# rapidsai/cugraph-gnn

Hardware: AMD Instinct MI355X
Metric: sampled-edges/sec (sample+renumber+feature-gather+SAGEConv fwd), ogbn-products-like fan-out [25, 10] (higher is better)
Workload: dtype int64 ids (int32 timed as a variant) + f32 features (SAGE lin_l/lin_r product: bf16x3-split MFMA, f32 accumulate); 1 GPU; ogbn-products-like RMAT: V=2449029, E=118462496 directed (CSR row_ptr i64 / col i64 replicated per GPU), feat fp32 [V,100], batch 1024/GPU, fan-out [25, 10], 2-layer SAGEConv(mean) 100-256-47 fwd, step = 8 call groups of 188 mini-batches; parallelism=dp1 (seeds sharded, no data-path collective)

## Files before the change

cugraph-gnn_amd/csrc/wg_sage_mfma.hip:

```cpp
#include "wg_sage_mfma_parts.hpp"

namespace wgamd {
namespace {
using namespace sage_mfma;

template <int TR>
__device__ __forceinline__ void consume_tile(const mfma_args& a, int64_t tile, const float* tile_lds, int cw, int lane,
                                             float* scratch)
{
  constexpr int RT = TR / 32;
  f32x16 c[RT][2];
#pragma unroll
  for (int rt = 0; rt < RT; rt++)
#pragma unroll
    for (int ct = 0; ct < 2; ct++)
#pragma unroll
      for (int i = 0; i < 16; i++) c[rt][ct][i] = 0.f;
  const int lm = lane & 31, lh = lane >> 5;
  const float* a_lane      = tile_lds + lm * a.SD + lh * 8;
  const float* b_lane = a.w_tiles + ((int64_t)(cw * 64 + lm)) * 16 + lh * 8;
  braw_t b0, b1;
  bfrag_t fb;
  araw_t<RT> raw;
  afrag_t<RT> fa;
  load_b(b0, b_lane, a.N, 0);
  for (int ks = 0; ks < a.KS; ks += 2) {
    load_a_raw<RT>(raw, a_lane, a.SD, ks);
    if (ks + 1 < a.KS) load_b(b1, b_lane, a.N, ks + 1);
    split_a<RT>(raw, fa);
    split_b(b0, fb);
    mma_frags<RT>(c, fa, fb);
    if (ks + 1 < a.KS) {
      load_a_raw<RT>(raw, a_lane, a.SD, ks + 1);
      if (ks + 2 < a.KS) load_b(b0, b_lane, a.N, ks + 2);
      split_a<RT>(raw, fa);
      split_b(b1, fb);
      mma_frags<RT>(c, fa, fb);
    }
  }
  epilogue<RT>(a, c, tile * TR, cw, lane, scratch);
}

template <int HEAD, int BODY, int VALU_PER>
__device__ __forceinline__ void mfma_valu_interleave()
{
#pragma unroll
  for (int i = 0; i < HEAD; i++) __builtin_amdgcn_sched_group_barrier(0x008, 1, 0);
#pragma unroll
  for (int i = 0; i < BODY; i++) {
    __builtin_amdgcn_sched_group_barrier(0x008, 1, 0);
    __builtin_amdgcn_sched_group_barrier(0x002, VALU_PER, 0);
  }
}

template <int RT, int AD, typename RawT = araw_t<RT>, typename LoadA>
__device__ __forceinline__ void consume_range(const mfma_args& a, f32x16 (&c)[RT][2], bfrag_t (&b)[3], int ks0, int ks1, int cw,
                                              int lane, LoadA load_a)
{
  const int lm = lane & 31, lh = lane >> 5;
  const int64_t b_plane_dw = (int64_t)a.KS * a.N * 8;
  const uint32_t* b_lane   = reinterpret_cast<const uint32_t*>(a.w_tiles) + ((int64_t)(cw * 64 + lm)) * 8 + lh * 4;
  RawT raw[AD];
  afrag_t<RT> fa[2];
  const int kl = ks1 - 1;
  load_a(raw[0], ks0);
  if constexpr (AD == 2) load_a(raw[1], ks0 + 1 < kl ? ks0 + 1 : kl);
  split_raw<RT>(raw[0], fa[0]);
  auto step = [&](auto I, int ks) {
    constexpr int i = decltype(I)::value;
    load_a(raw[i % AD], ks + AD < kl ? ks + AD : kl);
    int kb = ks + 2;
    kb     = kb >= a.KS ? kb - a.KS : kb;
    load_b_planes(b[(i + 2) % 3], b_lane, b_plane_dw, a.N, kb);
    mma_frags<RT>(c, fa[i & 1], b[i % 3]);
    split_raw<RT>(raw[(i + 1) % AD], fa[(i + 1) & 1]);
    mfma_valu_interleave<4, 6 * RT * 2 - 4, 5>();
    __builtin_amdgcn_sched_barrier(0);
  };
  int ks = ks0;
  for (; ks + 5 < ks1; ks += 6) {
    step(std::integral_constant<int, 0>{}, ks);
    step(std::integral_constant<int, 1>{}, ks + 1);
    step(std::integral_constant<int, 2>{}, ks + 2);
    step(std::integral_constant<int, 3>{}, ks + 3);
    step(std::integral_constant<int, 4>{}, ks + 4);
    step(std::integral_constant<int, 5>{}, ks + 5);
  }
  const int r = ks1 - ks;
  if (r > 0) step(std::integral_constant<int, 0>{}, ks);
  if (r > 1) step(std::integral_constant<int, 1>{}, ks + 1);
  if (r > 2) step(std::integral_constant<int, 2>{}, ks + 2);
  if (r > 3) step(std::integral_constant<int, 3>{}, ks + 3);
  if (r > 4) step(std::integral_constant<int, 4>{}, ks + 4);
  const int rot = (ks1 - ks0) % 3;
  if (rot == 1) {
    const bfrag_t t = b[0];
    b[0] = b[1], b[1] = b[2], b[2] = t;
  } else if (rot == 2) {
    const bfrag_t t = b[0];
    b[0] = b[2], b[2] = b[1], b[1] = t;
  }
}

constexpr int kPD = 2;
__host__ __device__ constexpr int b_slot(int ks) { return ks < kPD ? ks : kPD + (ks % kPD); }
__host__ __device__ constexpr int w_lds_ksteps(int FC)
{
#ifdef WG_NO_WLDS
  return 0;
#endif
  const int tiles = (2 * 64 * row_stride_dw(FC) + 16 + 4 * kScratchDw + 16) * 4;
  const int free_ = 160 * 1024 - tiles;
  const int ks    = free_ / (256 * 64);
  return ks < 0 ? 0 : (ks > 4 ? 4 : ks);
}

template <int TR, int FC>
struct static_consumer {
  static constexpr int RT = TR / 32, KSC = (2 * FC + 15) / 16, SD = row_stride_dw(FC);
  static constexpr int KL = TR == 64 ? w_lds_ksteps(FC) : 0;
  braw_t bb[2 * kPD];
  uint32_t b_lane_off;
  const float* w_lds;
  f32x16 c[RT][2];

  __device__ __forceinline__ void load_b_static(const mfma_args& a, braw_t& f, int ks) const
  {
#ifdef WG_ABL_NO_B
    return;
#endif
#ifdef WG_ABL_HALF_B
    if (ks & 1) return;
#endif
    if (ks >= KSC - KL) {
#pragma unroll
      for (int ct = 0; ct < 2; ct++)
#pragma unroll
        for (int h = 0; h < 2; h++)
          f.v[ct][h] = *reinterpret_cast<const f32x4*>(w_lds + (((ks - (KSC - KL)) * 2 + ct) * 2 + h) * 256);
      return;
    }
    const char* wb = reinterpret_cast<const char*>(a.w_tiles);
#pragma unroll
    for (int ct = 0; ct < 2; ct++) {
      const size_t at = ((size_t)ks * a.N + ct * 32) * 64 + b_lane_off;
      f.v[ct][0]      = *reinterpret_cast<const f32x4*>(wb + at);
      f.v[ct][1]      = *reinterpret_cast<const f32x4*>(wb + at + 16);
    }
  }

  __device__ __forceinline__ void prime(const mfma_args& a, int cw, int lane, float* w_lds_wave)
  {
    b_lane_off = (uint32_t)(((cw * 64 + (lane & 31)) * 16 + (lane >> 5) * 8) * 4);
    w_lds      = w_lds_wave + lane * 4;
    if constexpr (KL > 0) {
      const char* wb = reinterpret_cast<const char*>(a.w_tiles);
#pragma unroll
      for (int ks = KSC - KL; ks < KSC; ks++)
#pragma unroll
        for (int ct = 0; ct < 2; ct++)
#pragma unroll
          for (int h = 0; h < 2; h++)
            *reinterpret_cast<f32x4*>(const_cast<float*>(w_lds) + (((ks - (KSC - KL)) * 2 + ct) * 2 + h) * 256) =
              *reinterpret_cast<const f32x4*>(wb + ((size_t)ks * a.N + ct * 32) * 64 + b_lane_off + h * 16);
    }
#pragma unroll
    for (int j = 0; j < kPD; j++) load_b_static(a, bb[j], j);
  }

  __device__ __forceinline__ void multiply(const mfma_args& a, const float* tile_lds, int lane)
  {
#pragma unroll
    for (int rt = 0; rt < RT; rt++)
#pragma unroll
      for (int ct = 0; ct < 2; ct++)
#pragma unroll
        for (int i = 0; i < 16; i++) c[rt][ct][i] = 0.f;
    const float* a_lane = tile_lds + (lane & 31) * SD + (lane >> 5) * 8;
    araw_t<RT> raw;
    afrag_t<RT> fa[2];
    load_a_raw<RT>(raw, a_lane, SD, 0);
    split_a<RT>(raw, fa[0]);
#pragma unroll
    for (int ks = 0; ks < KSC; ks++) {
      if (ks + 1 < KSC) load_a_raw<RT>(raw, a_lane, SD, ks + 1);
      bfrag_t fb;
      split_b(bb[b_slot(ks)], fb);
      mma_frags<RT>(c, fa[ks & 1], fb);
      const int nk = ks + kPD;
      if (nk < KSC) load_b_static(a, bb[b_slot(nk)], nk);
      else load_b_static(a, bb[nk - KSC], nk - KSC);
      if (ks + 1 < KSC) split_a<RT>(raw, fa[(ks + 1) & 1]);
      __builtin_amdgcn_sched_barrier(0);
    }
  }
  __device__ __forceinline__ void store(const mfma_args& a, int64_t tile, int cw, int lane, float* scratch)
  {
    epilogue<RT>(a, c, tile * TR, cw, lane, scratch);
  }
};

template <typename IdT, int LG, int TR, int CW, bool OFF32, int FC, bool HALF = false, typename XT = float>
__global__ void __launch_bounds__((CW + kProducerWaves) * 64)
sage_layer_mfma_kernel(mfma_args a)
{
  static_assert(!HALF || FC == 0, "the half-tile mode runs the runtime-shape consumer");
  extern __shared__ __attribute__((aligned(16))) float lds[];
  const int tile_dw = TR * a.SD;
  uint32_t* ring = reinterpret_cast<uint32_t*>(lds + 2 * tile_dw + 16 + CW * kScratchDw) + 8;
  uint32_t first_ticket = kNoTile;
  if (threadIdx.x == 0 && (int64_t)blockIdx.x < (a.n_rows + TR - 1) / TR) first_ticket = (uint32_t)gridDim.x + atomicAdd(a.tickets, 1u);
  for (int i = threadIdx.x; i < 2 * tile_dw + 16; i += blockDim.x) lds[i] = 0.f;
  if (threadIdx.x == 0) ring[0] = blockIdx.x, ring[1] = first_ticket;
  __syncthreads();
  const int lane = threadIdx.x & 63;
  int wave = threadIdx.x >> 6;
  if (a.debug & 64) {
    uint32_t* keys = reinterpret_cast<uint32_t*>(lds + 2 * tile_dw + 16 + CW * kScratchDw);
    const int simd = (int)__builtin_amdgcn_s_getreg((1 << 11) | (4 << 6) | 4);
    if (lane == 0) keys[wave] = (uint32_t)(((simd & 1) * 2 + (simd >> 1)) * 16 + wave);
    __syncthreads();
    const uint32_t mine_key = keys[wave];
    int rank = 0;
#pragma unroll
    for (int w = 0; w < CW + kProducerWaves; w++) rank += keys[w] < mine_key ? 1 : 0;
    wave = __builtin_amdgcn_readfirstlane(rank);
    __syncthreads();
  }
  const uint32_t n_tiles = (uint32_t)((a.n_rows + TR - 1) / TR);
  const bool drawer      = wave == CW && lane == 0;
  auto draw              = [&](uint32_t known) {
    return known < n_tiles ? (uint32_t)gridDim.x + atomicAdd(a.tickets, 1u) : kNoTile;
  };
  auto ring_at = [&](int r) { return (uint32_t)__builtin_amdgcn_readfirstlane((int)ring[r]); };
  uint32_t t_prev = kNoTile, t_cur = ring_at(0);
  int r_next = 1;
  auto advance = [&](uint32_t t_next) {
    t_prev = t_cur, t_cur = t_next;
    r_next = r_next == 2 ? 0 : r_next + 1;
  };
  auto r_draw = [&] { return r_next == 2 ? 0 : r_next + 1; };
  auto stamp            = [&](int64_t n, int which) {
    if (a.stamps && blockIdx.x == 0 && lane == 0 && n < 64) a.stamps[(n * 8 + wave) * 2 + which] = __builtin_readcyclecounter();
  };

  if constexpr (HALF) {
    const int KSh = a.KS / 2;
    if (wave >= CW) {
      using P     = producer<IdT, LG, 32, OFF32, true, XT>;
      using off_t = typename P::off_t;
      constexpr int IT = P::IT, kNb = P::kNb, kDepth = P::kDepth;
      static_assert(TR == 64, "two 32-row sub-tiles per tile");
      P p(a, wave - CW, lane);
      bounds_t<IT> b_next;
      ids_t<IT> i_next;
      meta_t<IT, off_t> cur;
      typename P::raw_t buf[kDepth][kNb + 1];
      p.load_bounds(2 * (int64_t)t_cur, b_next);
      p.load_ids(2 * (int64_t)t_cur, b_next, i_next);
      p.finish(i_next, cur);
#pragma unroll
      for (int it = 0; it < kDepth - 1; it++) p.issue(cur, it, buf[it]);
      constexpr int kHalf = IT / 2;
      for (int n = 0;; n++) {
        const uint32_t t_next = ring_at(r_next);
        uint32_t drawn       = kNoTile;
        if (drawer && t_cur < n_tiles) drawn = draw(t_next);
        if (t_cur < n_tiles && !(a.debug & 2)) {
          float* tile_lds = lds + (n & 1) * tile_dw;
#pragma unroll
          for (int sub = 0; sub < 2; sub++) {
            const int64_t s_cur = 2 * (int64_t)t_cur + sub, s_next = sub == 0 ? s_cur + 1 : 2 * (int64_t)t_next;
            float* rows_lds = tile_lds + sub * 32 * a.SD;
            p.load_bounds(s_next, b_next);
#pragma unroll
            for (int it = 0; it < IT; it++) {
              if (it == kHalf) p.load_ids(s_next, b_next, i_next);
              if (it + kDepth - 1 < IT) p.issue(cur, it + kDepth - 1, buf[(it + kDepth - 1) % kDepth]);
              p.reduce_store(cur, it, buf[it % kDepth], rows_lds);
            }
            p.second_window(cur, rows_lds);
            p.long_rows(s_cur, cur, rows_lds);
            if (sub == 1 && drawer) ring[r_draw()] = drawn;
            p.finish(i_next, cur);
            if (sub == 0 || t_next < n_tiles) {
#pragma unroll
              for (int it = 0; it < kDepth - 1; it++) p.issue(cur, it, buf[it]);
            }
          }
        } else if (drawer) ring[r_draw()] = drawn;
        lds_barrier();
        if (t_cur >= n_tiles) break;
        advance(t_next);
      }
    } else {
      constexpr int RT = TR / 32;
      float* scratch = lds + 2 * tile_dw + 16 + wave * kScratchDw;
      f32x16 c[RT][2];
      bfrag_t b[3];
      {
        const uint32_t* b_lane =
          reinterpret_cast<const uint32_t*>(a.w_tiles) + ((int64_t)(wave * 64 + (lane & 31))) * 8 + (lane >> 5) * 4;
        load_b_planes(b[0], b_lane, (int64_t)a.KS * a.N * 8, a.N, 0);
        load_b_planes(b[1], b_lane, (int64_t)a.KS * a.N * 8, a.N, 1);
      }
      const IdT* src_ids = static_cast<const IdT*>(a.src_ids);
      for (int n = 0;; n++) {
        const uint32_t t_next = ring_at(r_next);
        if (n >= 1 && !(a.debug & 1)) {
          const int64_t row0 = (int64_t)t_prev * TR;
          constexpr int kEB = x16::row_elems<XT>::kBytes;
          using self_t      = typename std::conditional<kEB == 4, float, uint16_t>::type;
          const self_t* self_ptr[RT];
#pragma unroll
          for (int rt = 0; rt < RT; rt++) {
            const int64_t row  = row0 + rt * 32 + (lane & 31);
            const int64_t srow = a.self_rows[row < a.n_rows ? row : a.n_rows - 1];
            self_ptr[rt]       = reinterpret_cast<const self_t*>(reinterpret_cast<const char*>(a.x) + table_row<IdT>(src_ids, srow) * a.row_scale) +
                           (lane >> 5) * 8;
          }
#pragma unroll
          for (int rt = 0; rt < RT; rt++)
#pragma unroll
            for (int ct = 0; ct < 2; ct++)
#pragma unroll
              for (int i = 0; i < 16; i++) c[rt][ct][i] = 0.f;
          store_agg<TR, CW>(a, lds + ((n - 1) & 1) * tile_dw, row0, wave, lane);
          const float* a_lane = lds + ((n - 1) & 1) * tile_dw + (lane & 31) * a.SD + (lane >> 5) * 8;
          consume_range<RT, 1>(a, c, b, 0, KSh, wave, lane, [&](araw_t<RT>& f, int ks) { load_a_raw<RT>(f, a_lane, a.SD, ks); });
          if constexpr (kEB == 4) {
            consume_range<RT, 2>(a, c, b, KSh, a.KS, wave, lane, [&](araw_t<RT>& f, int ks) {
#pragma unroll
              for (int rt = 0; rt < RT; rt++) {
                const float* p = self_ptr[rt] + (ks - KSh) * 16;
                f.v[rt][0]     = *reinterpret_cast<const f32x4*>(p);
                f.v[rt][1]     = *reinterpret_cast<const f32x4*>(p + 4);
              }
            });
          } else {
            consume_range<RT, 2, araw16_t<XT, RT>>(a, c, b, KSh, a.KS, wave, lane, [&](araw16_t<XT, RT>& f, int ks) {
#pragma unroll
              for (int rt = 0; rt < RT; rt++)
                f.v[rt] = *reinterpret_cast<const x16::u32x4_a8*>(self_ptr[rt] + (ks - KSh) * 16);
            });
          }
          epilogue<RT>(a, c, row0, wave, lane, scratch);
        }
        lds_barrier();
        if (t_cur >= n_tiles) break;
        advance(t_next);
      }
    }
  } else if (wave >= CW) {
    if (a.debug & 16) __builtin_amdgcn_s_setprio(3);
    using P     = producer<IdT, LG, TR, OFF32, false, XT>;
    using off_t = typename P::off_t;
    constexpr int IT = P::IT, kNb = P::kNb, kDepth = P::kDepth;
    P p(a, wave - CW, lane);
    bounds_t<IT> b_next;
    ids_t<IT> i_next;
    meta_t<IT, off_t> cur;
    typename P::raw_t buf[kDepth][kNb + 1];
    {
      p.load_bounds(t_cur, b_next);
      p.load_ids(t_cur, b_next, i_next);
      p.finish(i_next, cur);
    }
#pragma unroll
    for (int it = 0; it < kDepth - 1; it++) p.issue(cur, it, buf[it]);
    constexpr int kHalf = IT / 2;
    for (int n = 0;; n++) {
      stamp(n, 0);
      const uint32_t t_next = ring_at(r_next);
      uint32_t drawn       = kNoTile;
      if (drawer && t_cur < n_tiles) drawn = draw(t_next);
      if (t_cur < n_tiles && !(a.debug & 2)) {
        float* tile_lds = lds + (n & 1) * tile_dw;
        p.load_bounds(t_next, b_next);
#pragma unroll
        for (int it = 0; it < IT; it++) {
          if (it == kHalf) p.load_ids(t_next, b_next, i_next);
          if (it + kDepth - 1 < IT) p.issue(cur, it + kDepth - 1, buf[(it + kDepth - 1) % kDepth]);
          p.reduce_store(cur, it, buf[it % kDepth], tile_lds);
        }
        p.second_window(cur, tile_lds);
        p.long_rows(t_cur, cur, tile_lds);
        if (drawer) ring[r_draw()] = drawn;
        p.finish(i_next, cur);
        if (t_next < n_tiles) {
#pragma unroll
          for (int it = 0; it < kDepth - 1; it++) p.issue(cur, it, buf[it]);
        }
      } else if (drawer) ring[r_draw()] = drawn;
      stamp(n, 1);
      lds_barrier();
      if (t_cur >= n_tiles) break;
      advance(t_next);
    }
  } else {
    if (a.debug & 32) __builtin_amdgcn_s_setprio(3);
    float* scratch = lds + 2 * tile_dw + 16 + wave * kScratchDw;
    if constexpr (FC > 0) {
      static_consumer<TR, FC> cons;
      cons.prime(a, wave, lane, lds + 2 * tile_dw + 16 + CW * kScratchDw + 16 + wave * (decltype(cons)::KL * 16 * 64));
      const bool late = (wave & 1) && !(a.debug & 128);
      int64_t pending = -1;
      for (int n = 0;; n++) {
        stamp(n, 0);
        const uint32_t t_next = ring_at(r_next);
        if (n >= 1 && !(a.debug & 1)) {
          const float* tile_lds = lds + ((n - 1) & 1) * tile_dw;
          store_agg<TR, CW>(a, tile_lds, (int64_t)t_prev * TR, wave, lane);
          if (late) {
            if (pending >= 0) cons.store(a, pending, wave, lane, scratch);
            cons.multiply(a, tile_lds, lane);
            pending = t_prev;
          } else {
            cons.multiply(a, tile_lds, lane);
            cons.store(a, t_prev, wave, lane, scratch);
          }
        }
        stamp(n, 1);
        lds_barrier();
        if (t_cur >= n_tiles) break;
        advance(t_next);
      }
      if (late && pending >= 0) cons.store(a, pending, wave, lane, scratch);
    } else {
      for (int n = 0;; n++) {
        const uint32_t t_next = ring_at(r_next);
        if (n >= 1 && !(a.debug & 1)) {
          store_agg<TR, CW>(a, lds + ((n - 1) & 1) * tile_dw, (int64_t)t_prev * TR, wave, lane);
          consume_tile<TR>(a, t_prev, lds + ((n - 1) & 1) * tile_dw, wave, lane, scratch);
        }
        lds_barrier();
        if (t_cur >= n_tiles) break;
        advance(t_next);
      }
    }
  }
  if (threadIdx.x == 0 && atomicAdd(a.tickets + 1, 1u) == gridDim.x - 1) {
    atomicExch(a.tickets, 0u);
    atomicExch(a.tickets + 1, 0u);
  }
}

__global__ void split_weight_kernel(const float* __restrict__ w_t, int64_t ldw, int K, int N, int KS, uint32_t* __restrict__ planes)
{
  const int64_t total = (int64_t)KS * N * 8;
  for (int64_t i = blockIdx.x * (int64_t)blockDim.x + threadIdx.x; i < total; i += (int64_t)gridDim.x * blockDim.x) {
    const int kk2 = (int)(i & 7);
    const int n   = (int)((i >> 3) % N);
    const int ks  = (int)((i >> 3) / N);
    const int k0  = ks * 16 + kk2 * 2;
    const float v0 = k0 < K ? w_t[(int64_t)k0 * ldw + n] : 0.f;
    const float v1 = k0 + 1 < K ? w_t[(int64_t)(k0 + 1) * ldw + n] : 0.f;
    uint32_t h0, m0, l0, h1, m1, l1;
    split3(v0, h0, m0, l0);
    split3(v1, h1, m1, l1);
    planes[i]             = pack_hi16(h0, h1);
    planes[total + i]     = pack_hi16(m0, m1);
    planes[2 * total + i] = pack_hi16(l0, l1);
  }
}

__global__ void tile_weight_kernel(const float* __restrict__ w_t, int64_t ldw, int K, int N, int KS, float* __restrict__ tiles)
{
  const int64_t total = (int64_t)KS * N * 16;
  for (int64_t i = blockIdx.x * (int64_t)blockDim.x + threadIdx.x; i < total; i += (int64_t)gridDim.x * blockDim.x) {
    const int kk = (int)(i & 15);
    const int n  = (int)((i >> 4) % N);
    const int ks = (int)((i >> 4) / N);
    const int k  = ks * 16 + kk;
    tiles[i]     = k < K ? w_t[(int64_t)k * ldw + n] : 0.f;
  }
}

__global__ void layer_weight_kernel(const float* __restrict__ w_l, int64_t ldl, const float* __restrict__ w_r, int64_t ldr,
                                    const float* __restrict__ bias, int F, int N, int Np, int KS, int half,
                                    void* __restrict__ planes_, float* __restrict__ bias_out)
{
  auto w_at = [&](int k, int n) -> float {
    if (n >= N || k >= 2 * F) return 0.f;
    return k < F ? w_l[(int64_t)n * ldl + k] : w_r[(int64_t)n * ldr + (k - F)];
  };
  const int64_t tid = blockIdx.x * (int64_t)blockDim.x + threadIdx.x, stride = (int64_t)gridDim.x * blockDim.x;
  if (bias_out)
    for (int64_t n = tid; n < Np; n += stride) bias_out[n] = (bias && n < N) ? bias[n] : 0.f;
  if (half) {
    uint32_t* planes    = static_cast<uint32_t*>(planes_);
    const int64_t total = (int64_t)KS * Np * 8;
    for (int64_t i = tid; i < total; i += stride) {
      const int kk2 = (int)(i & 7), n = (int)((i >> 3) % Np), ks = (int)((i >> 3) / Np);
      const int k0  = ks * 16 + kk2 * 2;
      uint32_t h0, m0, l0, h1, m1, l1;
      split3(w_at(k0, n), h0, m0, l0);
      split3(w_at(k0 + 1, n), h1, m1, l1);
      planes[i]             = pack_hi16(h0, h1);
      planes[total + i]     = pack_hi16(m0, m1);
      planes[2 * total + i] = pack_hi16(l0, l1);
    }
  } else {
    float* tiles        = static_cast<float*>(planes_);
    const int64_t total = (int64_t)KS * Np * 16;
    for (int64_t i = tid; i < total; i += stride) {
      const int kk = (int)(i & 15), n = (int)((i >> 4) % Np), ks = (int)((i >> 4) / Np);
      tiles[i]     = w_at(ks * 16 + kk, n);
    }
  }
}

constexpr int kSlotsPerBlock = 512;
__host__ inline uint32_t* ticket_slot(hipStream_t st)
{
  struct key_t {
    int dev;
    hipStream_t st;
    unsigned long long capture;
    bool operator<(const key_t& o) const { return std::tie(dev, st, capture) < std::tie(o.dev, o.st, o.capture); }
  };
  struct block_t {
    uint32_t* base;
    int used;
  };
  static std::mutex m;
  static std::map<key_t, uint32_t*> slot_of;
  static std::map<int, block_t> block_of;
  key_t key{0, st, 0};
  WG_HIP_CHECK(hipGetDevice(&key.dev));
  hipStreamCaptureStatus status = hipStreamCaptureStatusNone;
  if (st != nullptr) WG_HIP_CHECK(hipStreamGetCaptureInfo(st, &status, &key.capture));
  if (status != hipStreamCaptureStatusActive) key.capture = 0;
  std::lock_guard<std::mutex> g(m);
  auto it = slot_of.find(key);
  if (it != slot_of.end()) return it->second;
  block_t& b = block_of[key.dev];
  if (b.base == nullptr || b.used == kSlotsPerBlock) {
    hipStreamCaptureMode mode = hipStreamCaptureModeRelaxed;
    WG_HIP_CHECK(hipThreadExchangeStreamCaptureMode(&mode));
    void* p             = nullptr;
    const hipError_t e1 = hipMalloc(&p, kSlotsPerBlock * 2 * sizeof(uint32_t));
    const hipError_t e2 = e1 == hipSuccess ? hipMemset(p, 0, kSlotsPerBlock * 2 * sizeof(uint32_t)) : e1;
    WG_HIP_CHECK(hipThreadExchangeStreamCaptureMode(&mode));
    WG_HIP_CHECK(e1);
    WG_HIP_CHECK(e2);
    b = block_t{static_cast<uint32_t*>(p), 0};
  }
  uint32_t* slot = b.base + 2 * b.used++;
  slot_of.emplace(key, slot);
  return slot;
}

constexpr size_t kLdsBudget = 160 * 1024;
__host__ inline size_t lds_bytes(int F, int TR) { return (size_t)(2 * TR * row_stride_dw(F) + 16 + 4 * kScratchDw + 16) * 4; }
__host__ inline size_t lds_bytes_half(int F) { return (size_t)(2 * 64 * row_stride_half_dw(F) + 16 + 4 * kScratchDw + 16) * 4; }
__host__ inline bool use_half_tiles(int F)
{
  return F % 16 == 0 && lds_bytes(F, 64) > kLdsBudget && lds_bytes_half(F) <= kLdsBudget;
}

template <typename IdT, int LG, int CW, typename XT = float>
void launch_half(mfma_args a, hipStream_t st)
{
  const int cus         = stream_cu_count(st);
  a.tickets             = ticket_slot(st);
  a.SD                  = row_stride_half_dw(a.F);
  const int64_t n_tiles = (a.n_rows + 63) / 64;
  const size_t lds      = lds_bytes_half(a.F);
  const int grid        = (int)std::max<int64_t>(1, std::min<int64_t>(n_tiles, (int64_t)cus));
  auto go               = [&](auto kern) {
    WG_HIP_CHECK(hipFuncSetAttribute(reinterpret_cast<const void*>(kern), hipFuncAttributeMaxDynamicSharedMemorySize, (int)lds));
    kern<<<grid, (CW + kProducerWaves) * 64, lds, st>>>(a);
    WG_HIP_CHECK(hipGetLastError());
  };
  if (a.x_bytes != 0) go(sage_layer_mfma_kernel<IdT, LG, 64, CW, true, 0, true, XT>);
  else go(sage_layer_mfma_kernel<IdT, LG, 64, CW, false, 0, true, XT>);
}

template <typename IdT, int LG, int TR, int CW, int FC = 0, typename XT = float>
void launch(mfma_args a, hipStream_t st)
{
  const int cus         = stream_cu_count(st);
  a.tickets             = ticket_slot(st);
  const int64_t n_tiles = (a.n_rows + TR - 1) / TR;
  const size_t lds      = lds_bytes(a.F, TR) + (FC > 0 && TR == 64 ? (size_t)w_lds_ksteps(FC) * CW * 64 * 64 : 0);
  const int grid = (int)std::max<int64_t>(1, std::min<int64_t>(n_tiles, (int64_t)cus));
  auto go        = [&](auto kern) {
    if (lds > 64 * 1024)
      WG_HIP_CHECK(hipFuncSetAttribute(reinterpret_cast<const void*>(kern), hipFuncAttributeMaxDynamicSharedMemorySize, (int)lds));
    kern<<<grid, (CW + kProducerWaves) * 64, lds, st>>>(a);
    WG_HIP_CHECK(hipGetLastError());
  };
  if (a.x_bytes != 0) go(sage_layer_mfma_kernel<IdT, LG, TR, CW, true, FC, false, XT>);
  else go(sage_layer_mfma_kernel<IdT, LG, TR, CW, false, FC, false, XT>);
}

template <typename IdT, int LG, int TR, typename XT = float>
void launch_cw(const mfma_args& a, hipStream_t st)
{
  switch (a.N / 64) {
    case 1: launch<IdT, LG, TR, 1, 0, XT>(a, st); break;
    case 2: launch<IdT, LG, TR, 2, 0, XT>(a, st); break;
    default:
      if constexpr (LG == 32 && TR == 64) {
        if (a.F == 100) return launch<IdT, LG, TR, 4, 100, XT>(a, st);
        if (a.F == 128) return launch<IdT, LG, TR, 4, 128, XT>(a, st);
      }
      launch<IdT, LG, TR, 4, 0, XT>(a, st);
      break;
  }
}

template <typename IdT, int LG, typename XT = float>
void launch_tr(const mfma_args& a, hipStream_t st)
{
  if constexpr (LG <= 32) {
    launch_cw<IdT, LG, 64, XT>(a, st);
  } else {
    if (use_half_tiles(a.F) && !a.full_tiles) {
      switch (a.N / 64) {
        case 1: launch_half<IdT, LG, 1, XT>(a, st); break;
        case 2: launch_half<IdT, LG, 2, XT>(a, st); break;
        default: launch_half<IdT, LG, 4, XT>(a, st); break;
      }
    } else launch_cw<IdT, LG, 32, XT>(a, st);
  }
}

template <typename IdT, typename XT = float>
void launch_groups(const mfma_args& a, hipStream_t st)
{
  const int units = a.F / 4;
  if (units <= 8) launch_tr<IdT, 8, XT>(a, st);
  else if (units <= 16) launch_tr<IdT, 16, XT>(a, st);
  else if (units <= 32) launch_tr<IdT, 32, XT>(a, st);
  else launch_tr<IdT, 64, XT>(a, st);
}

}

namespace sage_mfma {
void launch_f16(const mfma_args& a, int ids_bytes, hipStream_t st);
void launch_bf16(const mfma_args& a, int ids_bytes, hipStream_t st);
#ifdef WG_SAGE_X16_TYPE
void WG_SAGE_X16_LAUNCH(const mfma_args& a, int ids_bytes, hipStream_t st)
{
  if (ids_bytes == 0) launch_groups<void, WG_SAGE_X16_TYPE>(a, st);
  else if (ids_bytes == 4) launch_groups<int32_t, WG_SAGE_X16_TYPE>(a, st);
  else launch_groups<int64_t, WG_SAGE_X16_TYPE>(a, st);
}
#endif
}
}

#if !defined(WG_MFMA_TUNE_HARNESS) && !defined(WG_SAGE_X16_TYPE)
extern "C" size_t wgamd_sage_weight_planes_bytes(int K, int N) { return (size_t)3 * ((K + 15) / 16) * (size_t)N * 32; }

extern "C" int wgamd_sage_layer_bf16x3_supported(int F, int N)
{
  return F > 0 && F % 4 == 0 && F <= 256 && (N == 64 || N == 128 || N == 256) && wgamd::lds_bytes(F, 32) <= wgamd::kLdsBudget;
}

extern "C" wholememory_error_code_t wgamd_sage_split_weight_bf16x3(const float* w_t, int64_t ldw, int K, int N, void* planes,
                                                                   void* stream)
{
  using namespace wgamd;
  return guarded("wgamd_sage_split_weight_bf16x3", [&] {
    WG_REQUIRE_INPUT(w_t && planes && K > 0 && N > 0 && ldw >= N, "bad weight");
    const int KS        = (K + 15) / 16;
    const int64_t total = (int64_t)KS * N * 16;
    const int grid      = (int)std::min<int64_t>((total + 255) / 256, 2048);
    if (K % 2 == 0 && use_half_tiles(K / 2))
      split_weight_kernel<<<grid, 256, 0, static_cast<hipStream_t>(stream)>>>(w_t, ldw, K, N, KS, static_cast<uint32_t*>(planes));
    else
      tile_weight_kernel<<<grid, 256, 0, static_cast<hipStream_t>(stream)>>>(w_t, ldw, K, N, KS, static_cast<float*>(planes));
    WG_HIP_CHECK(hipGetLastError());
  });
}

extern "C" int wgamd_sage_layer_uses_half_tiles(int F) { return wgamd::use_half_tiles(F) ? 1 : 0; }

extern "C" wholememory_error_code_t wgamd_sage_layer_weight_planes(const float* w_l, int64_t ldl, const float* w_r, int64_t ldr,
                                                                  const float* bias, int F, int N, int Np, void* planes,
                                                                  float* bias_out, int full_tiles, void* stream)
{
  using namespace wgamd;
  return guarded("wgamd_sage_layer_weight_planes", [&] {
    WG_REQUIRE_INPUT(w_l && w_r && planes && F > 0 && N > 0 && Np >= N && ldl >= F && ldr >= F, "bad weights");
    const int K = 2 * F, KS = (K + 15) / 16;
    const int half      = (use_half_tiles(F) && !full_tiles) ? 1 : 0;
    const int64_t total = (int64_t)KS * Np * 16;
    const int grid      = (int)std::min<int64_t>((total + 255) / 256, 2048);
    layer_weight_kernel<<<grid, 256, 0, static_cast<hipStream_t>(stream)>>>(w_l, ldl, w_r, ldr, bias, F, N, Np, KS, half, planes, bias_out);
    WG_HIP_CHECK(hipGetLastError());
  });
}

extern "C" wholememory_error_code_t wgamd_sage_layer_fused_bf16x3(const int* row_ptr, const int* col, int64_t n_rows,
                                                                  const float* x, int64_t ldx, int64_t x_rows, int F,
                                                                  const void* src_ids, wholememory_dtype_t src_ids_dtype,
                                                                  const int64_t* self_rows, int mean, const void* w_planes,
                                                                  int N, const float* bias, int relu, float* out, int64_t ldo,
                                                                  void* stream)
{
  return wgamd_sage_layer_fused_bf16x3_x_train(row_ptr, col, n_rows, x, WHOLEMEMORY_DT_FLOAT, ldx, x_rows, F, src_ids, src_ids_dtype,
                                               self_rows, mean, w_planes, N, bias, relu, out, ldo, nullptr, 0, stream);
}

extern "C" wholememory_error_code_t wgamd_sage_layer_fused_bf16x3_train(const int* row_ptr, const int* col, int64_t n_rows,
                                                                        const float* x, int64_t ldx, int64_t x_rows, int F,
                                                                        const void* src_ids, wholememory_dtype_t src_ids_dtype,
                                                                        const int64_t* self_rows, int mean, const void* w_planes,
                                                                        int N, const float* bias, int relu, float* out,
                                                                        int64_t ldo, float* agg_out, int64_t ld_agg, void* stream)
{
  return wgamd_sage_layer_fused_bf16x3_x_train(row_ptr, col, n_rows, x, WHOLEMEMORY_DT_FLOAT, ldx, x_rows, F, src_ids, src_ids_dtype,
                                               self_rows, mean, w_planes, N, bias, relu, out, ldo, agg_out, ld_agg, stream);
}

extern "C" int wgamd_sage_layer_x16_supported(int F, int N, wholememory_dtype_t x_dtype)
{
  return (x_dtype == WHOLEMEMORY_DT_FLOAT || x_dtype == WHOLEMEMORY_DT_HALF || x_dtype == WHOLEMEMORY_DT_BF16) &&
         wgamd_sage_layer_bf16x3_supported(F, N);
}

extern "C" wholememory_error_code_t wgamd_sage_layer_fused_bf16x3_x(const int* row_ptr, const int* col, int64_t n_rows,
                                                                    const void* x, wholememory_dtype_t x_dtype, int64_t ldx,
                                                                    int64_t x_rows, int F, const void* src_ids,
                                                                    wholememory_dtype_t src_ids_dtype, const int64_t* self_rows,
// ... 60 lines not shown
```

cugraph-gnn_amd/csrc/wg_sage_mfma_parts.hpp:

```cpp
#pragma once
#include <algorithm>
#include <cstdlib>
#include <map>
#include <mutex>
#include <tuple>
#include <type_traits>

#include "wg_common.hpp"
#include "wgamd_ext.h"
#include "wg_x16.hpp"

namespace wgamd {
namespace sage_mfma {

using f32x4  = __attribute__((ext_vector_type(4))) float;
using f32x16 = __attribute__((ext_vector_type(16))) float;
using u32x4  = __attribute__((ext_vector_type(4))) uint32_t;
using bf16x8 = __attribute__((ext_vector_type(8))) __bf16;

#ifndef WG_MFMA_PRODUCTS
#define WG_MFMA_PRODUCTS 6
#endif
#ifndef WG_MFMA_DEPTH
#define WG_MFMA_DEPTH 2
// ... 234 lines not shown
  {
    if constexpr (k < kNb + (HALF ? 0 : 1)) {
      issue_one<k>(m, it, v);
      issue_all<k + 1>(m, it, v);
    }
  }
  template <int k>
  __device__ __forceinline__ void issue_one(const meta_t<IT, off_t>& m, int it, raw_t* v) const
  {
    static_assert(!HALF || k < kNb, "no self slot in half-tile mode");
    if constexpr (OFF32) {
      if constexpr (k < kNb) {
        const uint32_t off = (uint32_t)group_lane<k>((int)m.src[it]);
        v[k] = bload(k < m.d[it] ? off + f0c * kEB : a.x_bytes);
      } else {
        v[kNb] = bload(m.d[it] >= 0 ? (uint32_t)m.self[it] + f0c * kEB : a.x_bytes);
      }
    } else {
      const char* xb = reinterpret_cast<const char*>(a.x);
      if constexpr (k < kNb) {
        const int lo = group_lane<k>((int)(m.src[it] & 0xffffffff));
        const int hi = group_lane<k>((int)((int64_t)m.src[it] >> 32));
        int64_t off  = ((int64_t)hi << 32) | (uint32_t)lo;
        off          = k < m.d[it] ? off : (int64_t)0;
        v[k]         = gload(xb + off + f0c * kEB);
      } else {
        v[kNb] = gload(xb + (m.d[it] >= 0 ? (int64_t)m.self[it] : (int64_t)0) + f0c * kEB);
      }
    }
  }
  __device__ __forceinline__ void reduce_store(const meta_t<IT, off_t>& m, int it, const raw_t* v, float* tile_lds) const
  {
    const int deg = m.d[it];
    f32x4 acc     = {0.f, 0.f, 0.f, 0.f};
#pragma unroll
    for (int k = 0; k < kNb; k++) {
      if constexpr (OFF32) acc += E::f32(v[k]);
      else acc += k < deg ? E::f32(v[k]) : f32x4{0.f, 0.f, 0.f, 0.f};
    }
    if (a.mean && deg > 0 && deg <= kNb) acc *= __frcp_rn((float)deg);
    if (live) {
      float* prow = tile_lds + (group + it * kGroups) * a.SD;
      *reinterpret_cast<f32x4*>(prow + f0) = acc;
      if constexpr (!HALF) {
        f32x4 self = E::f32(v[kNb]);
        if constexpr (!OFF32) self = deg >= 0 ? self : f32x4{0.f, 0.f, 0.f, 0.f};
        *reinterpret_cast<f32x4*>(prow + a.F + f0) = self;
      }
    }
  }
  static constexpr int kW2 = LG >= 32 ? 16 : (LG > kNb ? LG - kNb : 0);
  __device__ __forceinline__ void second_window(const meta_t<IT, off_t>& m, float* tile_lds) const
  {
    if constexpr (kW2 > 0) {
#pragma unroll
      for (int it = 0; it < IT; it++) {
        const int deg = m.d[it];
        if (__ballot(deg > kNb) == 0ull) continue;
        const bool mine = live && deg > kNb;
        raw_t v[kW2];
#pragma unroll
        for (int k = 0; k < kW2; k++) {
          const int kk = kNb + k;
          if constexpr (OFF32) {
            const uint32_t off = (uint32_t)__shfl((int)m.src[it], gbase | kk, 64);
            v[k] = bload(kk < deg ? off + f0c * kEB : a.x_bytes);
          } else {
            const int lo = __shfl((int)(m.src[it] & 0xffffffff), gbase | kk, 64);
            const int hi = __shfl((int)((int64_t)m.src[it] >> 32), gbase | kk, 64);
            int64_t off  = ((int64_t)hi << 32) | (uint32_t)lo;
            off          = kk < deg ? off : (int64_t)0;
            v[k]         = gload(reinterpret_cast<const char*>(a.x) + off + f0c * kEB);
          }
        }
        float* prow = tile_lds + (group + it * kGroups) * a.SD + f0;
        f32x4 acc   = {0.f, 0.f, 0.f, 0.f};
        if (mine) acc = *reinterpret_cast<const f32x4*>(prow);
#pragma unroll
        for (int k = 0; k < kW2; k++) {
          if constexpr (OFF32) acc += E::f32(v[k]);
          else acc += kNb + k < deg ? E::f32(v[k]) : f32x4{0.f, 0.f, 0.f, 0.f};
        }
        if (mine) {
          if (a.mean && deg <= kNb + kW2) acc *= __frcp_rn((float)deg);
          *reinterpret_cast<f32x4*>(prow) = acc;
        }
      }
    }
  }
  static constexpr int kLongUnroll = 8;
  __device__ __forceinline__ void long_rows(int64_t tile, const meta_t<IT, off_t>& m, float* tile_lds) const
  {
    long_rows_from<kNb + kW2, kLongUnroll>(tile, m, tile_lds);
  }
  template <int kStart, int kUnroll>
  __device__ __forceinline__ void long_rows_from(int64_t tile, const meta_t<IT, off_t>& m, float* tile_lds) const
  {
    const IdT* src_ids = static_cast<const IdT*>(a.src_ids);
#pragma unroll
    for (int it = 0; it < IT; it++) {
      const int deg = m.d[it];
      if (__ballot(deg > kStart) == 0ull) continue;
      const bool mine    = live && deg > kStart;
      const int64_t row  = row_of(tile, it);
      const int64_t rowc = row < a.n_rows ? row : a.n_rows - 1;
      const int s        = a.row_ptr[rowc];
      float* prow        = tile_lds + (group + it * kGroups) * a.SD + f0;
      f32x4 acc          = {0.f, 0.f, 0.f, 0.f};
      if (mine) acc = *reinterpret_cast<const f32x4*>(prow);
      int maxdeg = deg > kStart ? deg : 0;
#pragma unroll
      for (int dd = 32; dd >= LG; dd >>= 1) maxdeg = max(maxdeg, __shfl_xor(maxdeg, dd, 64));
      for (int c0 = kStart; c0 < maxdeg; c0 += LG) {
        const int64_t my_src = (deg > kStart && c0 + sub < deg) ? table_row<IdT>(src_ids, (int64_t)a.col[s + c0 + sub]) : 0;
        const int chunk      = min(LG, maxdeg - c0);
        for (int j0 = 0; j0 < chunk; j0 += kUnroll) {
          raw_t v[kUnroll];
#pragma unroll
          for (int u = 0; u < kUnroll; u++) {
            const int j        = j0 + u;
            const int src_lane = gbase | (j & (LG - 1));
            const int lo       = __shfl((int)(my_src & 0xffffffff), src_lane, 64);
            const int hi       = __shfl((int)(my_src >> 32), src_lane, 64);
            const int64_t rr   = (mine && j < chunk && c0 + j < deg) ? (((int64_t)hi << 32) | (uint32_t)lo) : (int64_t)0;
            v[u] = gload(reinterpret_cast<const char*>(a.x) + rr * a.row_scale + f0c * kEB);
          }
#pragma unroll
          for (int u = 0; u < kUnroll; u++) {
            const int j = j0 + u;
            acc += (mine && j < chunk && c0 + j < deg) ? E::f32(v[u]) : f32x4{0.f, 0.f, 0.f, 0.f};
          }
        }
      }
      if (mine) {
        if (a.mean) acc *= __frcp_rn((float)deg);
        *reinterpret_cast<f32x4*>(prow) = acc;
      }
    }
  }
};

template <int RT>
struct araw_t {
  f32x4 v[RT][2];
};
template <typename XT, int RT>
struct araw16_t {
  x16::u32x4 v[RT];
};
template <int RT>
struct afrag_t {
  u32x4 v[RT][3];
};
struct bfrag_t {
  u32x4 v[2][3];
};
struct braw_t {
  f32x4 v[2][2];
};

template <int RT>
__device__ __forceinline__ void load_a_raw(araw_t<RT>& f, const float* a_lane, int sd, int ks)
{
#pragma unroll
  for (int rt = 0; rt < RT; rt++) {
    f.v[rt][0] = *reinterpret_cast<const f32x4*>(a_lane + rt * 32 * sd + ks * 16);
    f.v[rt][1] = *reinterpret_cast<const f32x4*>(a_lane + rt * 32 * sd + ks * 16 + 4);
  }
}
template <int RT>
__device__ __forceinline__ void split_a(const araw_t<RT>& r, afrag_t<RT>& f)
{
#pragma unroll
  for (int rt = 0; rt < RT; rt++) {
#ifdef WG_ABL_NO_SPLIT
#pragma unroll
    for (int j = 0; j < 4; j++) {
      f.v[rt][0][j] = __float_as_uint(r.v[rt][0][j]);
      f.v[rt][1][j] = __float_as_uint(r.v[rt][1][j]);
      f.v[rt][2][j] = __float_as_uint(r.v[rt][0][j]);
    }
    continue;
#endif
    uint32_t h[8], m[8], l[8];
#pragma unroll
    for (int i = 0; i < 4; i++) {
      split3(r.v[rt][0][i], h[i], m[i], l[i]);
      split3(r.v[rt][1][i], h[4 + i], m[4 + i], l[4 + i]);
    }
#pragma unroll
    for (int j = 0; j < 4; j++) {
      f.v[rt][0][j] = pack_hi16(h[2 * j], h[2 * j + 1]);
      f.v[rt][1][j] = pack_hi16(m[2 * j], m[2 * j + 1]);
      f.v[rt][2][j] = pack_hi16(l[2 * j], l[2 * j + 1]);
    }
  }
}
template <int RT>
__device__ __forceinline__ void split_raw(const araw_t<RT>& r, afrag_t<RT>& f)
{
  split_a<RT>(r, f);
}
template <int RT, typename XT>
__device__ __forceinline__ void split_raw(const araw16_t<XT, RT>& r, afrag_t<RT>& f)
{
  araw_t<RT> w;
#pragma unroll
  for (int rt = 0; rt < RT; rt++) {
    w.v[rt][0] = x16::to_f32x4<XT>(x16::u32x2{r.v[rt][0], r.v[rt][1]});
    w.v[rt][1] = x16::to_f32x4<XT>(x16::u32x2{r.v[rt][2], r.v[rt][3]});
  }
  split_a<RT>(w, f);
}
__device__ __forceinline__ void load_b(braw_t& f, const float* b_lane, int n_cols, int ks)
{
#pragma unroll
  for (int ct = 0; ct < 2; ct++) {
    const float* p = b_lane + ((int64_t)ks * n_cols + ct * 32) * 16;
    f.v[ct][0]     = *reinterpret_cast<const f32x4*>(p);
    f.v[ct][1]     = *reinterpret_cast<const f32x4*>(p + 4);
  }
}
__device__ __forceinline__ void load_b_planes(bfrag_t& f, const uint32_t* b_lane, int64_t b_plane_dw, int n_cols, int ks)
{
#ifdef WG_ABL_NO_B
  return;
#endif
#pragma unroll
  for (int ct = 0; ct < 2; ct++)
#pragma unroll
    for (int p = 0; p < 3; p++)
      f.v[ct][p] = *reinterpret_cast<const u32x4*>(b_lane + p * b_plane_dw + ((int64_t)ks * n_cols + ct * 32) * 8);
}
__device__ __forceinline__ void split_b(const braw_t& r, bfrag_t& f)
{
#pragma unroll
  for (int ct = 0; ct < 2; ct++) {
    uint32_t h[8], m[8], l[8];
#pragma unroll
    for (int i = 0; i < 4; i++) {
      split3(r.v[ct][0][i], h[i], m[i], l[i]);
      split3(r.v[ct][1][i], h[4 + i], m[4 + i], l[4 + i]);
    }
#pragma unroll
    for (int j = 0; j < 4; j++) {
      f.v[ct][0][j] = pack_hi16(h[2 * j], h[2 * j + 1]);
      f.v[ct][1][j] = pack_hi16(m[2 * j], m[2 * j + 1]);
      f.v[ct][2][j] = pack_hi16(l[2 * j], l[2 * j + 1]);
    }
  }
}

template <int RT>
__device__ __forceinline__ void mma_frags(f32x16 (&c)[RT][2], const afrag_t<RT>& fa, const bfrag_t& fb)
{
  constexpr int pa[6] = {2, 0, 1, 1, 0, 0};
  constexpr int pb[6] = {0, 2, 1, 0, 1, 0};
#pragma unroll
  for (int t = 0; t < WG_MFMA_PRODUCTS; t++)
#pragma unroll
    for (int rt = 0; rt < RT; rt++)
#pragma unroll
      for (int ct = 0; ct < 2; ct++)
        c[rt][ct] = __builtin_amdgcn_mfma_f32_32x32x16_bf16(__builtin_bit_cast(bf16x8, fa.v[rt][pa[t]]),
                                                            __builtin_bit_cast(bf16x8, fb.v[ct][pb[t]]), c[rt][ct], 0, 0, 0);
}

constexpr int kScratchDw = 8 * 64;

template <int RT>
__device__ __forceinline__ void epilogue(const mfma_args& a, f32x16 (&c)[RT][2], int64_t row0, int cw, int lane, float* scratch)
{
  const int lm = lane & 31, lh = lane >> 5;
  float bj[2];
#pragma unroll
  for (int ct = 0; ct < 2; ct++) bj[ct] = a.bias ? a.bias[cw * 64 + ct * 32 + lm] : 0.f;
  if (a.debug & 4) {
    if (c[0][0][0] == 12345.678f) a.out[0] = c[0][1][3] + c[RT - 1][1][5];
    return;
  }
  const bool full = row0 + RT * 32 <= a.n_rows;
  const int rl = lane >> 4, cl = (lane & 15) * 4;
  float* obase = a.out + (row0 + rl) * a.ldo + cw * 64 + cl;
#pragma unroll
  for (int rt = 0; rt < RT; rt++)
#pragma unroll
    for (int g = 0; g < 4; g++) {
#pragma unroll
      for (int ct = 0; ct < 2; ct++)
#pragma unroll
        for (int jj = 0; jj < 4; jj++) {
          const float v = c[rt][ct][4 * g + jj] + bj[ct];
          scratch[(jj + 4 * lh) * 64 + ct * 32 + lm] = a.relu ? fmaxf(v, 0.f) : v;
        }
#pragma unroll
      for (int pass = 0; pass < 2; pass++) {
        const f32x4 v = *reinterpret_cast<const f32x4*>(scratch + (rl + 4 * pass) * 64 + cl);
        const int r   = rt * 32 + 8 * g + 4 * pass;
        if (full || row0 + r + rl < a.n_rows) *reinterpret_cast<f32x4*>(obase + (int64_t)r * a.ldo) = v;
      }
    }
}

template <int TR, int CW>
__device__ __forceinline__ void store_agg(const mfma_args& a, const float* tile_lds, int64_t row0, int cw, int lane)
{
  if (a.agg_out == nullptr) return;
  constexpr int kRows = TR / CW;
  const int q_row = a.F >> 2, total = kRows * q_row;
  for (int i = lane; i < total; i += 64) {
    const int r = i / q_row, q = i - r * q_row;
    const int64_t row = row0 + cw * kRows + r;
    if (row < a.n_rows)
      *reinterpret_cast<f32x4*>(a.agg_out + row * a.ld_agg + q * 4) =
        *reinterpret_cast<const f32x4*>(tile_lds + (cw * kRows + r) * a.SD + q * 4);
  }
}

}
}
```

Before: 5.644 billion sampled-edges/s.

## Split the output-head SAGE tile across four consumer waves with one accumulator each

When the half-tile launcher is asked for a single consumer wave, it now launches four consumer waves instead. Each wave owns one 32x32 quadrant of the 64x64 output tile, so its row and column offsets, B-fragment width and MFMA loop change accordingly. Fragment types and helpers are templated on the column-tile count, and a dedicated quadrant epilogue plus a different MFMA/VALU interleave are added for the one-accumulator case. The aim is to stop the narrow output layer's GEMM from being serialized on one wave. The cost is duplicated weight and A-row loads across waves, and more waves competing for block resources.

```diff
diff --git a/cugraph-gnn_amd/csrc/wg_sage_mfma.hip b/cugraph-gnn_amd/csrc/wg_sage_mfma.hip
--- a/cugraph-gnn_amd/csrc/wg_sage_mfma.hip
+++ b/cugraph-gnn_amd/csrc/wg_sage_mfma.hip
@@ -53,13 +53,13 @@
   }
 }
 
-template <int RT, int AD, typename RawT = araw_t<RT>, typename LoadA>
-__device__ __forceinline__ void consume_range(const mfma_args& a, f32x16 (&c)[RT][2], bfrag_t (&b)[3], int ks0, int ks1, int cw,
-                                              int lane, LoadA load_a)
+template <int RT, int AD, typename RawT = araw_t<RT>, int CT, typename LoadA>
+__device__ __forceinline__ void consume_range(const mfma_args& a, f32x16 (&c)[RT][CT], bfrag_n<CT> (&b)[3], int ks0, int ks1,
+                                              int col0, int lane, LoadA load_a)
 {
   const int lm = lane & 31, lh = lane >> 5;
   const int64_t b_plane_dw = (int64_t)a.KS * a.N * 8;
-  const uint32_t* b_lane   = reinterpret_cast<const uint32_t*>(a.w_tiles) + ((int64_t)(cw * 64 + lm)) * 8 + lh * 4;
+  const uint32_t* b_lane   = reinterpret_cast<const uint32_t*>(a.w_tiles) + ((int64_t)(col0 + lm)) * 8 + lh * 4;
   RawT raw[AD];
   afrag_t<RT> fa[2];
   const int kl = ks1 - 1;
@@ -74,7 +74,8 @@
     load_b_planes(b[(i + 2) % 3], b_lane, b_plane_dw, a.N, kb);
     mma_frags<RT>(c, fa[i & 1], b[i % 3]);
     split_raw<RT>(raw[(i + 1) % AD], fa[(i + 1) & 1]);
-    mfma_valu_interleave<4, 6 * RT * 2 - 4, 5>();
+    if constexpr (RT * CT == 1) mfma_valu_interleave<0, 6, 9>();
+    else mfma_valu_interleave<4, 6 * RT * CT - 4, 5>();
     __builtin_amdgcn_sched_barrier(0);
   };
   int ks = ks0;
@@ -94,10 +95,10 @@
   if (r > 4) step(std::integral_constant<int, 4>{}, ks + 4);
   const int rot = (ks1 - ks0) % 3;
   if (rot == 1) {
-    const bfrag_t t = b[0];
+    const bfrag_n<CT> t = b[0];
     b[0] = b[1], b[1] = b[2], b[2] = t;
   } else if (rot == 2) {
-    const bfrag_t t = b[0];
+    const bfrag_n<CT> t = b[0];
     b[0] = b[2], b[2] = b[1], b[1] = t;
   }
 }
@@ -200,11 +201,12 @@
   }
 };
 
-template <typename IdT, int LG, int TR, int CW, bool OFF32, int FC, bool HALF = false, typename XT = float>
+template <typename IdT, int LG, int TR, int CW, bool OFF32, int FC, bool HALF = false, typename XT = float, bool HEAD = false>
 __global__ void __launch_bounds__((CW + kProducerWaves) * 64)
 sage_layer_mfma_kernel(mfma_args a)
 {
   static_assert(!HALF || FC == 0, "the half-tile mode runs the runtime-shape consumer");
+  static_assert(!HEAD || (HALF && CW == 4 && TR == 64), "one accumulator per wave: four waves over a 64 x 64 tile in half-tile mode");
   extern __shared__ __attribute__((aligned(16))) float lds[];
   const int tile_dw = TR * a.SD;
   uint32_t* ring = reinterpret_cast<uint32_t*>(lds + 2 * tile_dw + 16 + CW * kScratchDw) + 8;
@@ -294,13 +296,15 @@
         advance(t_next);
       }
     } else {
-      constexpr int RT = TR / 32;
+      constexpr int RT = HEAD ? 1 : TR / 32, CT = HEAD ? 1 : 2;
+      const int rt0    = HEAD ? wave >> 1 : 0;
+      const int col0   = HEAD ? (wave & 1) * 32 : wave * 64;
       float* scratch = lds + 2 * tile_dw + 16 + wave * kScratchDw;
-      f32x16 c[RT][2];
-      bfrag_t b[3];
+      f32x16 c[RT][CT];
+      bfrag_n<CT> b[3];
       {
         const uint32_t* b_lane =
-          reinterpret_cast<const uint32_t*>(a.w_tiles) + ((int64_t)(wave * 64 + (lane & 31))) * 8 + (lane >> 5) * 4;
+          reinterpret_cast<const uint32_t*>(a.w_tiles) + ((int64_t)(col0 + (lane & 31))) * 8 + (lane >> 5) * 4;
         load_b_planes(b[0], b_lane, (int64_t)a.KS * a.N * 8, a.N, 0);
         load_b_planes(b[1], b_lane, (int64_t)a.KS * a.N * 8, a.N, 1);
       }
@@ -314,7 +318,7 @@
           const self_t* self_ptr[RT];
 #pragma unroll
           for (int rt = 0; rt < RT; rt++) {
-            const int64_t row  = row0 + rt * 32 + (lane & 31);
+            const int64_t row  = row0 + (rt0 + rt) * 32 + (lane & 31);
             const int64_t srow = a.self_rows[row < a.n_rows ? row : a.n_rows - 1];
             self_ptr[rt]       = reinterpret_cast<const self_t*>(reinterpret_cast<const char*>(a.x) + table_row<IdT>(src_ids, srow) * a.row_scale) +
                            (lane >> 5) * 8;
@@ -322,14 +326,14 @@
 #pragma unroll
           for (int rt = 0; rt < RT; rt++)
 #pragma unroll
-            for (int ct = 0; ct < 2; ct++)
+            for (int ct = 0; ct < CT; ct++)
 #pragma unroll
               for (int i = 0; i < 16; i++) c[rt][ct][i] = 0.f;
           store_agg<TR, CW>(a, lds + ((n - 1) & 1) * tile_dw, row0, wave, lane);
-          const float* a_lane = lds + ((n - 1) & 1) * tile_dw + (lane & 31) * a.SD + (lane >> 5) * 8;
-          consume_range<RT, 1>(a, c, b, 0, KSh, wave, lane, [&](araw_t<RT>& f, int ks) { load_a_raw<RT>(f, a_lane, a.SD, ks); });
+          const float* a_lane = lds + ((n - 1) & 1) * tile_dw + (rt0 * 32 + (lane & 31)) * a.SD + (lane >> 5) * 8;
+          consume_range<RT, 1>(a, c, b, 0, KSh, col0, lane, [&](araw_t<RT>& f, int ks) { load_a_raw<RT>(f, a_lane, a.SD, ks); });
           if constexpr (kEB == 4) {
-            consume_range<RT, 2>(a, c, b, KSh, a.KS, wave, lane, [&](araw_t<RT>& f, int ks) {
+            consume_range<RT, 2>(a, c, b, KSh, a.KS, col0, lane, [&](araw_t<RT>& f, int ks) {
 #pragma unroll
               for (int rt = 0; rt < RT; rt++) {
                 const float* p = self_ptr[rt] + (ks - KSh) * 16;
@@ -338,13 +342,14 @@
               }
             });
           } else {
-            consume_range<RT, 2, araw16_t<XT, RT>>(a, c, b, KSh, a.KS, wave, lane, [&](araw16_t<XT, RT>& f, int ks) {
+            consume_range<RT, 2, araw16_t<XT, RT>>(a, c, b, KSh, a.KS, col0, lane, [&](araw16_t<XT, RT>& f, int ks) {
 #pragma unroll
               for (int rt = 0; rt < RT; rt++)
                 f.v[rt] = *reinterpret_cast<const x16::u32x4_a8*>(self_ptr[rt] + (ks - KSh) * 16);
             });
           }
-          epilogue<RT>(a, c, row0, wave, lane, scratch);
+          if constexpr (HEAD) epilogue_head(a, c[0][0], row0 + rt0 * 32, col0, lane, scratch);
+          else epilogue<RT>(a, c, row0, wave, lane, scratch);
         }
         lds_barrier();
         if (t_cur >= n_tiles) break;
@@ -559,9 +564,11 @@
   return F % 16 == 0 && lds_bytes(F, 64) > kLdsBudget && lds_bytes_half(F) <= kLdsBudget;
 }
 
-template <typename IdT, int LG, int CW, typename XT = float>
+template <typename IdT, int LG, int NW, typename XT = float>
 void launch_half(mfma_args a, hipStream_t st)
 {
+  constexpr bool HEAD = NW == 1;
+  constexpr int CW    = HEAD ? 4 : NW;
   const int cus         = stream_cu_count(st);
   a.tickets             = ticket_slot(st);
   a.SD                  = row_stride_half_dw(a.F);
@@ -573,8 +580,8 @@
     kern<<<grid, (CW + kProducerWaves) * 64, lds, st>>>(a);
     WG_HIP_CHECK(hipGetLastError());
   };
-  if (a.x_bytes != 0) go(sage_layer_mfma_kernel<IdT, LG, 64, CW, true, 0, true, XT>);
-  else go(sage_layer_mfma_kernel<IdT, LG, 64, CW, false, 0, true, XT>);
+  if (a.x_bytes != 0) go(sage_layer_mfma_kernel<IdT, LG, 64, CW, true, 0, true, XT, HEAD>);
+  else go(sage_layer_mfma_kernel<IdT, LG, 64, CW, false, 0, true, XT, HEAD>);
 }
 
 template <typename IdT, int LG, int TR, int CW, int FC = 0, typename XT = float>
diff --git a/cugraph-gnn_amd/csrc/wg_sage_mfma_parts.hpp b/cugraph-gnn_amd/csrc/wg_sage_mfma_parts.hpp
--- a/cugraph-gnn_amd/csrc/wg_sage_mfma_parts.hpp
+++ b/cugraph-gnn_amd/csrc/wg_sage_mfma_parts.hpp
@@ -410,9 +410,11 @@
 struct afrag_t {
   u32x4 v[RT][3];
 };
-struct bfrag_t {
-  u32x4 v[2][3];
-};
+template <int CT>
+struct bfrag_n {
+  u32x4 v[CT][3];
+};
+using bfrag_t = bfrag_n<2>;
 struct braw_t {
   f32x4 v[2][2];
 };
@@ -479,13 +481,14 @@
     f.v[ct][1]     = *reinterpret_cast<const f32x4*>(p + 4);
   }
 }
-__device__ __forceinline__ void load_b_planes(bfrag_t& f, const uint32_t* b_lane, int64_t b_plane_dw, int n_cols, int ks)
+template <int CT>
+__device__ __forceinline__ void load_b_planes(bfrag_n<CT>& f, const uint32_t* b_lane, int64_t b_plane_dw, int n_cols, int ks)
 {
 #ifdef WG_ABL_NO_B
   return;
 #endif
 #pragma unroll
-  for (int ct = 0; ct < 2; ct++)
+  for (int ct = 0; ct < CT; ct++)
 #pragma unroll
     for (int p = 0; p < 3; p++)
       f.v[ct][p] = *reinterpret_cast<const u32x4*>(b_lane + p * b_plane_dw + ((int64_t)ks * n_cols + ct * 32) * 8);
@@ -509,8 +512,8 @@
   }
 }
 
-template <int RT>
-__device__ __forceinline__ void mma_frags(f32x16 (&c)[RT][2], const afrag_t<RT>& fa, const bfrag_t& fb)
+template <int RT, int CT>
+__device__ __forceinline__ void mma_frags(f32x16 (&c)[RT][CT], const afrag_t<RT>& fa, const bfrag_n<CT>& fb)
 {
   constexpr int pa[6] = {2, 0, 1, 1, 0, 0};
   constexpr int pb[6] = {0, 2, 1, 0, 1, 0};
@@ -519,7 +522,7 @@
 #pragma unroll
     for (int rt = 0; rt < RT; rt++)
 #pragma unroll
-      for (int ct = 0; ct < 2; ct++)
+      for (int ct = 0; ct < CT; ct++)
         c[rt][ct] = __builtin_amdgcn_mfma_f32_32x32x16_bf16(__builtin_bit_cast(bf16x8, fa.v[rt][pa[t]]),
                                                             __builtin_bit_cast(bf16x8, fb.v[ct][pb[t]]), c[rt][ct], 0, 0, 0);
 }
@@ -558,6 +561,29 @@
         if (full || row0 + r + rl < a.n_rows) *reinterpret_cast<f32x4*>(obase + (int64_t)r * a.ldo) = v;
       }
     }
+}
+
+__device__ __forceinline__ void epilogue_head(const mfma_args& a, const f32x16& c, int64_t row0, int col0, int lane, float* scratch)
+{
+  const int lm = lane & 31, lh = lane >> 5;
+  const float bj = a.bias ? a.bias[col0 + lm] : 0.f;
+  if (a.debug & 4) {
+    if (c[0] == 12345.678f) a.out[0] = c[3] + c[5];
+    return;
+  }
+  const bool full = row0 + 32 <= a.n_rows;
+  const int rl = lane >> 3, cl = (lane & 7) * 4;
+  float* obase = a.out + (row0 + rl) * a.ldo + col0 + cl;
+#pragma unroll
+  for (int g = 0; g < 4; g++) {
+#pragma unroll
+    for (int jj = 0; jj < 4; jj++) {
+      const float v = c[4 * g + jj] + bj;
+      scratch[(jj + 4 * lh) * 32 + lm] = a.relu ? fmaxf(v, 0.f) : v;
+    }
+    const f32x4 v = *reinterpret_cast<const f32x4*>(scratch + rl * 32 + cl);
+    if (full || row0 + 8 * g + rl < a.n_rows) *reinterpret_cast<f32x4*>(obase + (int64_t)(8 * g) * a.ldo) = v;
+  }
 }
 
 template <int TR, int CW>
```

Result: faster. 5.704 billion sampled-edges/s, median of 6 (+1.1%).
